# mpasha3/trips-py

Hardware: AMD Instinct MI355X
Metric: krylov_iters_per_sec (higher is better)
Workload: dtype f32; 1 GPU; blur4096_cgls; image=4096x4096 fp32, psf=Gaussian 9x9 sigma=(3,3), reflect, solver=CGLS (trips.solvers.CGLS semantics, tol=0), noise=1% Gaussian, parallelism=single

## Files before the change

trips_py_amd/csrc/blur2d.hip:

```cpp
#include "trk_internal.h"
#include <hip/hip_ext.h>

#include <cmath>
#include <cstdlib>
#include <type_traits>
#include <vector>

using namespace trk;

namespace {

constexpr int NT = 256;
constexpr int TW = 128;
constexpr int TH = 32;

typedef float f4 __attribute__((ext_vector_type(4)));

__host__ __device__ constexpr int rup4(int v) { return (v + 3) & ~3; }

__device__ __forceinline__ int reflect(int i, int n) {
  if ((unsigned)i < (unsigned)n) return i;
  const int p = 2 * n;
  i %= p;
  if (i < 0) i += p;
  return (i >= n) ? (p - 1 - i) : i;
}

enum Bc : int { BC_REFLECT = 0, BC_CONSTANT = 1, BC_NEAREST = 2, BC_MIRROR = 3, BC_WRAP = 4 };

template <int BC>
__device__ __forceinline__ int bmap(int i, int n) {
  if constexpr (BC == BC_REFLECT) {
    return reflect(i, n);
  } else {
    if ((unsigned)i < (unsigned)n) return i;
    if constexpr (BC == BC_CONSTANT) {
      return -1;
    } else if constexpr (BC == BC_NEAREST) {
      return i < 0 ? 0 : n - 1;
    } else if constexpr (BC == BC_WRAP) {
      i %= n;
      return i < 0 ? i + n : i;
    } else {
      if (n == 1) return 0;
      const int p = 2 * n - 2;
      i %= p;
      if (i < 0) i += p;
      return (i >= n) ? (p - i) : i;
    }
  }
}

template <int BC>
__device__ __forceinline__ float bload(const float* row, int j, int n) {
  const int g = bmap<BC>(j, n);
  if constexpr (BC == BC_CONSTANT)
    if (g < 0) return 0.f;
  return row[g];
}

template <class F>
int bc_dispatch(int bc, F&& f) {
  switch (bc) {
    case BC_CONSTANT: return f(std::integral_constant<int, BC_CONSTANT>{});
    case BC_NEAREST: return f(std::integral_constant<int, BC_NEAREST>{});
    case BC_MIRROR: return f(std::integral_constant<int, BC_MIRROR>{});
    case BC_WRAP: return f(std::integral_constant<int, BC_WRAP>{});
    default: return f(std::integral_constant<int, BC_REFLECT>{});
  }
}

struct BlurImpl {
  int nx, ny, kh, kw;
  int bc;
  bool separable;
  bool tiled;
  float* w_dev[2];
  float* sep_dev[2];
};

template <int KH, int KW, bool SEP, bool SUMSQ, int BC = BC_REFLECT>
__global__ __launch_bounds__(NT, (SEP && KH <= 9) ? 4 : 2) void k_blur_strip(const float* __restrict__ x, int64_t ldx, float* __restrict__ y,
                                                   int64_t ldy, int nx, int ny, const float* __restrict__ wts,
                                                   double* __restrict__ partials, int strips_x, int rows_per_band) {
  constexpr int T = KH - 1 - KH / 2;
  constexpr int L = KW - 1 - KW / 2;
  constexpr int R = KW / 2;
  constexpr int LP = rup4(L), RP = rup4(R);
  constexpr int SW = TW + LP + RP;
  constexpr int RING = TH + KH - 1;
  constexpr int OFF = LP - L;
  constexpr int NV = (OFF + KW + 3 + 3) / 4;
  constexpr int SW4 = SW / 4;
  constexpr int NPF = (TH * SW4 + NT - 1) / NT;

  __shared__ f4 S4[RING * SW4];
  float* const S = reinterpret_cast<float*>(S4);
  __shared__ double red[NT / 64];

  const int sj = blockIdx.x % strips_x, band = blockIdx.x / strips_x;
  const int j0 = sj * TW;
  const int i_begin = band * rows_per_band;
  const int i_end = (i_begin + rows_per_band < nx) ? i_begin + rows_per_band : nx;
  x += (int64_t)blockIdx.y * ldx;
  y += (int64_t)blockIdx.y * ldy;

  const bool fast = ((ny & 3) == 0) && ((reinterpret_cast<uintptr_t>(x) & 15u) == 0);

  auto load_group = [&](int rel, int c4) -> f4 {
    const int gi = bmap<BC>(i_begin - T + rel, nx);
    if constexpr (BC == BC_CONSTANT)
      if (gi < 0) return (f4){0.f, 0.f, 0.f, 0.f};
    const int gc = j0 - LP + 4 * c4;
    const float* row = x + (int64_t)gi * ny;
    if (fast && gc >= 0 && gc + 3 < ny) return *reinterpret_cast<const f4*>(row + gc);
    return (f4){bload<BC>(row, gc, ny), bload<BC>(row, gc + 1, ny), bload<BC>(row, gc + 2, ny), bload<BC>(row, gc + 3, ny)};
  };

  auto load_direct = [&](int rel0, int count) {
    for (int idx = threadIdx.x; idx < count * SW4; idx += NT) {
      const int r = idx / SW4, c4 = idx - r * SW4;
      S4[((rel0 + r) % RING) * SW4 + c4] = load_group(rel0 + r, c4);
    }
  };

  float wr[SEP ? KW : 1], wc[SEP ? KH : 1];
  if (SEP) {
#pragma unroll
    for (int b = 0; b < KW; ++b) wr[b] = wts[b];
#pragma unroll
    for (int a = 0; a < KH; ++a) wc[a] = wts[KW + a];
  }

  const int tx = threadIdx.x & 31, ty = threadIdx.x >> 5;
  const int gj = j0 + 4 * tx;
  const bool vec_ok = ((ny & 3) == 0) && ((reinterpret_cast<uintptr_t>(y) & 15u) == 0) && (j0 + TW <= ny);
  double ss = 0.0;

  load_direct(0, RING);
  int rb = 0;
  for (int i0 = i_begin; i0 < i_end; i0 += TH) {
    const int rel_base = i0 - i_begin;
    const bool has_next = (i0 + TH < i_end);
    __syncthreads();

    f4 pf[NPF];
#pragma unroll
    for (int q = 0; q < NPF; ++q) pf[q] = (f4){0.f, 0.f, 0.f, 0.f};
    if (has_next) {
#pragma unroll
      for (int q = 0; q < NPF; ++q) {
        const int idx = threadIdx.x + q * NT;
        if (idx < TH * SW4) {
          const int r = idx / SW4, c4 = idx - r * SW4;
          pf[q] = load_group(rel_base + RING + r, c4);
        }
      }
    }

    float acc[4][4];
#pragma unroll
    for (int rr = 0; rr < 4; ++rr)
#pragma unroll
      for (int c = 0; c < 4; ++c) acc[rr][c] = 0.f;
#pragma unroll
    for (int a = 0; a < KH + 3; ++a) {
      int slot = rb + 4 * ty + a;
      if (slot >= RING) slot -= RING;
      float v[NV * 4];
#pragma unroll
      for (int q = 0; q < NV; ++q) {
        const f4 t = S4[slot * SW4 + tx + q];
        v[4 * q] = t[0];
        v[4 * q + 1] = t[1];
        v[4 * q + 2] = t[2];
        v[4 * q + 3] = t[3];
      }
      if (SEP) {
        float h[4] = {0.f, 0.f, 0.f, 0.f};
#pragma unroll
        for (int b = 0; b < KW; ++b)
#pragma unroll
          for (int c = 0; c < 4; ++c) h[c] = fmaf(wr[b], v[OFF + c + b], h[c]);
#pragma unroll
        for (int rr = 0; rr < 4; ++rr) {
          if (a - rr >= 0 && a - rr < KH) {
            const float w = wc[a - rr];
#pragma unroll
            for (int c = 0; c < 4; ++c) acc[rr][c] = fmaf(w, h[c], acc[rr][c]);
          }
        }
      } else {
#pragma unroll
        for (int rr = 0; rr < 4; ++rr) {
          if (a - rr >= 0 && a - rr < KH) {
#pragma unroll
            for (int b = 0; b < KW; ++b) {
              const float w = wts[(a - rr) * KW + b];
#pragma unroll
              for (int c = 0; c < 4; ++c) acc[rr][c] = fmaf(w, v[OFF + c + b], acc[rr][c]);
            }
          }
        }
      }
    }

    if (vec_ok) {
#pragma unroll
      for (int rr = 0; rr < 4; ++rr) {
        const int gi = i0 + 4 * ty + rr;
        if (gi < i_end) {
          *reinterpret_cast<f4*>(y + (int64_t)gi * ny + gj) = (f4){acc[rr][0], acc[rr][1], acc[rr][2], acc[rr][3]};
          if (SUMSQ)
            ss += (double)acc[rr][0] * acc[rr][0] + (double)acc[rr][1] * acc[rr][1] +
                  (double)acc[rr][2] * acc[rr][2] + (double)acc[rr][3] * acc[rr][3];
        }
      }
    } else {
#pragma unroll
      for (int rr = 0; rr < 4; ++rr) {
        const int gi = i0 + 4 * ty + rr;
        if (gi < i_end) {
#pragma unroll
          for (int c = 0; c < 4; ++c)
            if (gj + c < ny) {
              y[(int64_t)gi * ny + gj + c] = acc[rr][c];
              if (SUMSQ) ss += (double)acc[rr][c] * acc[rr][c];
            }
        }
      }
    }

    if (has_next) {
      __syncthreads();
#pragma unroll
      for (int q = 0; q < NPF; ++q) {
        const int idx = threadIdx.x + q * NT;
        if (idx < TH * SW4) {
          const int r = idx / SW4, c4 = idx - r * SW4;
          S4[((rel_base + RING + r) % RING) * SW4 + c4] = pf[q];
        }
      }
      rb += TH;
      if (rb >= RING) rb -= RING;
    }
  }
  if (SUMSQ) {
    ss = block_sum<NT>(ss, red);
    if (threadIdx.x == 0) partials[(size_t)blockIdx.y * gridDim.x + blockIdx.x] = ss;
  }
}

typedef unsigned int u4 __attribute__((ext_vector_type(4)));
typedef float f2 __attribute__((ext_vector_type(2)));

__host__ __device__ constexpr int gcd_c(int a, int b) { return b == 0 ? a : gcd_c(b, a % b); }
__host__ __device__ constexpr int lcm_c(int a, int b) { return a / gcd_c(a, b) * b; }
__host__ __device__ constexpr int pmod(int a, int m) { return ((a % m) + m) % m; }

constexpr int SPAN = 256;

struct SlideFuse {
  const float* x2;
  float* comb;
  double sign;
  ScalarSrc num, den;
};

struct SlideEpi {
  const float* z;
  Coef a, b;
};

enum Rc : int { RC_NONE = 0, RC_NORM = 1, RC_RATIO = 2 };
struct SlideRatio {
  const float* z;
  float* out;
  ScalarSrc num, den;
  float sign;
  int on_z, pub_den;
  double* pub;
};

template <int KH, int KW, int D, bool SUMSQ, bool FUSE, bool EPI = false, int BC = BC_REFLECT, int RC = RC_NONE>
__global__ __launch_bounds__(64) void k_blur_slide(const float* __restrict__ x, int64_t ldx, float* __restrict__ y,
                                                   int64_t ldy, int nx, int ny, const float* __restrict__ wts,
                                                   double* __restrict__ partials, int spans_x, int nbands,
                                                   int rows_per_band, SlideFuse fz, int nt_store, SlideEpi ep = SlideEpi{},
                                                   SlideRatio rq = SlideRatio{}) {
  static_assert(RC == RC_NONE || !FUSE, "the recompute forms take one operand");
  static_assert(RC != RC_NORM || (SUMSQ && !EPI), "RC_NORM: the sum of squares alone");
  static_assert(RC != RC_RATIO || (EPI && !SUMSQ), "RC_RATIO: an epilogue form without a sum");
  constexpr int T = KH - 1 - KH / 2;
  constexpr int Lh = KW - 1 - KW / 2;
  constexpr int OFFC = 4 - Lh;
  constexpr int U = lcm_c(KH, D);
  static_assert(Lh <= 4 && KW / 2 <= 4, "sliding kernel handles halos of at most one 4-column group");

  int band, span;
  {
    const int id = blockIdx.x, total = nbands * spans_x;
    const int xcd = id & 7, local = id >> 3;
    const int t = xcd * (total >> 3) + min(xcd, total & 7) + local;
    band = t / spans_x;
    span = t - band * spans_x;
  }
  x += (int64_t)blockIdx.y * ldx;
  y += (int64_t)blockIdx.y * ldy;
  const int i_begin = band * rows_per_band;
  const int i_end = (i_begin + rows_per_band < nx) ? i_begin + rows_per_band : nx;
  const int lane = threadIdx.x;
  const int c0 = span * SPAN + 4 * lane;
  const bool active = c0 < ny;
  const int cc = active ? c0 : ny - 4;
  const int cl = (BC == BC_WRAP && c0 == 0) ? ny - 4 : (cc >= 4) ? cc - 4 : 0;
  const int cr = (BC == BC_WRAP && c0 + 4 == ny) ? 0 : (cc + 8 <= ny) ? cc + 4 : ny - 4;
  const bool ledge = (c0 == 0), redge = (c0 + 4 == ny);
  const bool edge_span = (span == 0) || ((span + 1) * SPAN >= ny);

  const unsigned img_bytes = (unsigned)nx * (unsigned)ny * 4u;
  const auto rin = __builtin_amdgcn_make_buffer_rsrc((void*)x, 0, img_bytes, 0x00020000);
  const auto rout = __builtin_amdgcn_make_buffer_rsrc((void*)(RC == RC_RATIO ? rq.out : y), 0, img_bytes, 0x00020000);
  const auto rin2 = __builtin_amdgcn_make_buffer_rsrc((void*)(FUSE ? fz.x2 : x), 0, img_bytes, 0x00020000);
  const auto rcomb = __builtin_amdgcn_make_buffer_rsrc((void*)(FUSE ? fz.comb : y), 0, img_bytes, 0x00020000);
  float cb = 0.f;
  if (FUSE) cb = (fz.sign == 0.0) ? 0.f : (float)(fz.sign * scalar_from_wave(fz.num, threadIdx.x) / scalar_from_wave(fz.den, threadIdx.x));
  const int vl = cl * 4, vr = cr * 4;
  const int vc = cc * 4;
  const int vst = c0 * 4;

  const bool up = (band & 1) != 0;
  float wr[KW], wc[KH];
#pragma unroll
  for (int b = 0; b < KW; ++b) wr[b] = wts[b];
#pragma unroll
  for (int a = 0; a < KH; ++a) wc[a] = up ? wts[KW + KH - 1 - a] : wts[KW + a];

  const int band_rows = i_end - i_begin;
  const int total = ((band_rows + KH - 1 + U - 1) / U) * U;
  const int rowbytes = ny * 4;
  const int dir = up ? -1 : 1;
  const int first = up ? (i_end - 1 + KH / 2) : (i_begin - T);
  const int last = first + dir * (total - 1);
  const bool interior = (first >= 0) && (first < nx) && (last >= 0) && (last < nx);
  const int ofirst = up ? (i_end - 1) : i_begin;

  f4 pL[D], pC[D], pR[D];
  f4 qL[FUSE ? D : 1], qC[FUSE ? D : 1], qR[FUSE ? D : 1];
  auto issue = [&](int t, int slot) {
    int gi = first + dir * t;
    if (!interior) gi = bmap<BC>(gi, nx);
    if constexpr (BC == BC_CONSTANT) {
      if (gi < 0) {
        const f4 z = (f4){0.f, 0.f, 0.f, 0.f};
        pL[slot] = pC[slot] = pR[slot] = z;
        if (FUSE) qL[slot] = qC[slot] = qR[slot] = z;
        return;
      }
    }
    const int so = gi * rowbytes;
    pL[slot] = __builtin_bit_cast(f4, __builtin_amdgcn_raw_buffer_load_b128(rin, vl, so, 0));
    pC[slot] = __builtin_bit_cast(f4, __builtin_amdgcn_raw_buffer_load_b128(rin, vc, so, 0));
    pR[slot] = __builtin_bit_cast(f4, __builtin_amdgcn_raw_buffer_load_b128(rin, vr, so, 0));
    if (FUSE) {
      qL[slot] = __builtin_bit_cast(f4, __builtin_amdgcn_raw_buffer_load_b128(rin2, vl, so, 0));
      qC[slot] = __builtin_bit_cast(f4, __builtin_amdgcn_raw_buffer_load_b128(rin2, vc, so, 0));
      qR[slot] = __builtin_bit_cast(f4, __builtin_amdgcn_raw_buffer_load_b128(rin2, vr, so, 0));
    }
  };
#pragma unroll
  for (int d = 0; d < D; ++d) issue(d, d);
  float ea = 1.f, eb = 0.f;
  f4 zq[EPI ? D : 1];
  const auto rz = __builtin_amdgcn_make_buffer_rsrc((void*)(RC == RC_RATIO ? rq.z : (EPI && ep.z) ? ep.z : x), 0, img_bytes, 0x00020000);
  const bool has_z = RC == RC_RATIO || (EPI && ep.z != nullptr);
  auto issue_z = [&](int o, int slot) {
    const int oc = o < band_rows - 1 ? o : band_rows - 1;
    zq[slot] = __builtin_bit_cast(f4, __builtin_amdgcn_raw_buffer_load_b128(rz, vc, (ofirst + dir * oc) * rowbytes, 0));
  };
  if constexpr (RC == RC_RATIO) {
#pragma unroll
    for (int d = 0; d < D; ++d) issue_z(d, d);
    const double qn = scalar_from_wave(rq.num, lane), qd = scalar_from_wave(rq.den, lane);
    const float c = rq.sign * (float)(qn / qd);
    ea = rq.on_z ? 1.f : c;
    eb = rq.on_z ? c : 1.f;
    if (blockIdx.x == 0 && blockIdx.y == 0 && lane == 0 && rq.pub) *rq.pub = rq.pub_den ? qd : qn;
  } else if (EPI) {
    ea = (float)coef_eval(ep.a);
    eb = has_z ? (float)coef_eval(ep.b) : 0.f;
    if (has_z) {
#pragma unroll
      for (int d = 0; d < D; ++d) issue_z(d, d);
    }
  }

  f2 acc[KH][2];
  double ss = 0.0;
  float qacc = 0.f;

  auto block = [&](int t0, auto guard_tag) {
    constexpr bool GUARD = decltype(guard_tag)::value;
#pragma unroll
    for (int u = 0; u < U; ++u) {
      const int t = t0 + u;
      const int slot = u % D;
      f4 Lv = pL[slot], Cv = pC[slot], Rv = pR[slot];
      if (FUSE) {
        Lv = Lv + cb * qL[slot];
        Cv = Cv + cb * qC[slot];
        Rv = Rv + cb * qR[slot];
        const int graw = first + dir * t;
        if (graw >= i_begin && graw < i_end && active)
          __builtin_amdgcn_raw_buffer_store_b128(__builtin_bit_cast(u4, Cv), rcomb, vst + graw * rowbytes, 0, 0);
      }
      if (!GUARD || t + D < total) issue(t + D, slot);
      if constexpr (BC == BC_REFLECT) {
        if (edge_span) {
          const f4 rev = (f4){Cv[3], Cv[2], Cv[1], Cv[0]};
          if (ledge) Lv = rev;
          if (redge) Rv = rev;
        }
      } else if constexpr (BC != BC_WRAP) {
        if (edge_span) {
          f4 le, re;
          if constexpr (BC == BC_CONSTANT) {
            le = re = (f4){0.f, 0.f, 0.f, 0.f};
          } else if constexpr (BC == BC_NEAREST) {
            le = (f4){Cv[0], Cv[0], Cv[0], Cv[0]};
            re = (f4){Cv[3], Cv[3], Cv[3], Cv[3]};
          } else {
            le = (f4){Rv[0], Cv[3], Cv[2], Cv[1]};
            re = (f4){Cv[2], Cv[1], Cv[0], Lv[3]};
          }
          if (ledge) Lv = le;
          if (redge) Rv = re;
        }
      }
      const float v[12] = {Lv[0], Lv[1], Lv[2], Lv[3], Cv[0], Cv[1], Cv[2], Cv[3], Rv[0], Rv[1], Rv[2], Rv[3]};
      float h0 = 0.f, h1 = 0.f, h2 = 0.f, h3 = 0.f;
#pragma unroll
      for (int b = 0; b < KW; ++b) {
        h0 = fmaf(wr[b], v[OFFC + b], h0);
        h1 = fmaf(wr[b], v[OFFC + b + 1], h1);
        h2 = fmaf(wr[b], v[OFFC + b + 2], h2);
        h3 = fmaf(wr[b], v[OFFC + b + 3], h3);
      }
      const f2 hlo = {h0, h1}, hhi = {h2, h3};
#pragma unroll
      for (int a = 0; a < KH; ++a) {
        const int k = pmod(u - a, KH);
        if (a == 0) {
          acc[k][0] = wc[0] * hlo;
          acc[k][1] = wc[0] * hhi;
        } else {
          acc[k][0] = wc[a] * hlo + acc[k][0];
          acc[k][1] = wc[a] * hhi + acc[k][1];
        }
      }
      const int o = t - (KH - 1);
      if (!GUARD || (o >= 0 && o < band_rows)) {
        const int kd = pmod(u - (KH - 1), KH);
        f4 out = (f4){acc[kd][0][0], acc[kd][0][1], acc[kd][1][0], acc[kd][1][1]};
        if (EPI) {
          const int zs = pmod(u - (KH - 1), D);
          if constexpr (RC == RC_RATIO) {
            const f4 zv = zq[zs];
            if (rq.on_z) {
#pragma unroll
              for (int e = 0; e < 4; ++e) out[e] = fmaf(eb, zv[e], out[e]);
            } else {
#pragma unroll
              for (int e = 0; e < 4; ++e) out[e] = fmaf(ea, out[e], zv[e]);
            }
            issue_z(o + D, zs);
          } else if (has_z) {
            const f4 zv = zq[zs];
#pragma unroll
            for (int e = 0; e < 4; ++e) out[e] = fmaf(ea, out[e], eb * zv[e]);
            issue_z(o + D, zs);
          } else {
#pragma unroll
            for (int e = 0; e < 4; ++e) out[e] = ea * out[e];
          }
        }
        if (active) {
          if constexpr (RC != RC_NORM) {
            if (nt_store & 1)
              __builtin_amdgcn_raw_buffer_store_b128(__builtin_bit_cast(u4, out), rout, vst + (ofirst + dir * o) * rowbytes, 0, 2);
            else
              __builtin_amdgcn_raw_buffer_store_b128(__builtin_bit_cast(u4, out), rout, vst + (ofirst + dir * o) * rowbytes, 0, 0);
          }
          if (SUMSQ) qacc = fmaf(out[0], out[0], fmaf(out[1], out[1], fmaf(out[2], out[2], fmaf(out[3], out[3], qacc))));
        }
      }
      if (SUMSQ && (u & 3) == 3) {
        ss += (double)qacc;
        qacc = 0.f;
      }
    }
  };
  block(0, std::true_type{});
  int t0 = U;
  for (; t0 + U < total; t0 += U) block(t0, std::false_type{});
  if (t0 < total) block(t0, std::true_type{});
  if (SUMSQ) ss += (double)qacc;
  if (SUMSQ) {
    ss = wave_sum(ss);
    if (lane == 0) partials[(size_t)blockIdx.y * gridDim.x + blockIdx.x] = ss;
  }
}

template <bool SUMSQ, int BC = BC_REFLECT>
__global__ __launch_bounds__(NT) void k_blur_generic(const float* __restrict__ x, int64_t ldx, float* __restrict__ y,
                                                     int64_t ldy, int nx, int ny, int kh, int kw,
                                                     const float* __restrict__ w, double* __restrict__ partials) {
  __shared__ double red[NT / 64];
  const int T = kh - 1 - kh / 2, L = kw - 1 - kw / 2;
  x += (int64_t)blockIdx.y * ldx;
  y += (int64_t)blockIdx.y * ldy;
  const int64_t npix = (int64_t)nx * ny;
  double ss = 0.0;
  for (int64_t idx = (int64_t)blockIdx.x * NT + threadIdx.x; idx < npix; idx += (int64_t)gridDim.x * NT) {
    const int i = (int)(idx / ny), j = (int)(idx - (int64_t)i * ny);
    float acc = 0.f;
    for (int a = 0; a < kh; ++a) {
      const int gi = bmap<BC>(i - T + a, nx);
      if constexpr (BC == BC_CONSTANT)
        if (gi < 0) continue;
      const float* row = x + (int64_t)gi * ny;
      for (int b = 0; b < kw; ++b) acc = fmaf(w[a * kw + b], bload<BC>(row, j - L + b, ny), acc);
    }
    y[idx] = acc;
    if (SUMSQ) ss += (double)acc * acc;
  }
  if (SUMSQ) {
    ss = block_sum<NT>(ss, red);
    if (threadIdx.x == 0) partials[(size_t)blockIdx.y * gridDim.x + blockIdx.x] = ss;
  }
}

inline void strip_grid(int nx, int ny, int batch, int* strips_x, int* rows_per_band, int* nband) {
  const int sx = ceil_div(ny, TW), steps = ceil_div(nx, TH);
  int want = (4 * cu_count()) / (sx * (batch > 0 ? batch : 1));
  if (want < 1) want = 1;
  if (want > steps) want = steps;
  const int steps_per_band = ceil_div(steps, want);
  *strips_x = sx;
  *rows_per_band = steps_per_band * TH;
  *nband = ceil_div(nx, *rows_per_band);
}

template <int K, int BC>
int launch_strip(const BlurImpl* im, int tr, const float* x, int64_t ldx, float* y, int64_t ldy, int batch,
                 double* part, int strips_x, int rows_per_band, int nband, hipStream_t s) {
  dim3 grid(strips_x * nband, batch), block(NT);
  const float* w = im->separable ? im->sep_dev[tr] : im->w_dev[tr];
#define BL(SEP, SS) \
  hipLaunchKernelGGL((k_blur_strip<K, K, SEP, SS, BC>), grid, block, 0, s, x, ldx, y, ldy, im->nx, im->ny, w, part, strips_x, rows_per_band)
  if (im->separable) { if (part) BL(true, true); else BL(true, false); }
  else               { if (part) BL(false, true); else BL(false, false); }
#undef BL
  TRK_LAUNCH_CHECK();
  return TRK_OK;
}

template <int K, int D, int BC>
int launch_slide(const BlurImpl* im, int tr, const float* x, int64_t ldx, float* y, int64_t ldy, int batch,
                 double* part, int spans_x, int nbands, int rows_per_band, hipStream_t s, hipEvent_t ev0, hipEvent_t ev1,
                 const SlideFuse* fuse = nullptr, const SlideEpi* epi = nullptr) {
  dim3 grid(spans_x * nbands, batch), block(64);
  const float* w = im->sep_dev[tr];
  const int nts = stream_nontemporal((int64_t)im->nx * im->ny);
  if (fuse) {
    hipExtLaunchKernelGGL((k_blur_slide<K, K, D, true, true, false, BC>), grid, block, 0, s, ev0, ev1, 0, x, ldx, y, ldy, im->nx, im->ny, w, part, spans_x, nbands, rows_per_band, *fuse, nts, SlideEpi{}, SlideRatio{});
    TRK_LAUNCH_CHECK();
    return TRK_OK;
  }
  const SlideFuse nofuse{nullptr, nullptr, 0.0, {nullptr, 0}, {nullptr, 0}};
  if (epi) {
    if (part)
      hipExtLaunchKernelGGL((k_blur_slide<K, K, D, true, false, true, BC>), grid, block, 0, s, ev0, ev1, 0, x, ldx, y, ldy, im->nx, im->ny, w, part, spans_x, nbands, rows_per_band, nofuse, nts, *epi, SlideRatio{});
    else
      hipExtLaunchKernelGGL((k_blur_slide<K, K, D, false, false, true, BC>), grid, block, 0, s, ev0, ev1, 0, x, ldx, y, ldy, im->nx, im->ny, w, part, spans_x, nbands, rows_per_band, nofuse, nts, *epi, SlideRatio{});
    TRK_LAUNCH_CHECK();
    return TRK_OK;
  }
  if (part)
    hipExtLaunchKernelGGL((k_blur_slide<K, K, D, true, false, false, BC>), grid, block, 0, s, ev0, ev1, 0, x, ldx, y, ldy, im->nx, im->ny, w, part, spans_x, nbands, rows_per_band, nofuse, nts, SlideEpi{}, SlideRatio{});
  else
    hipExtLaunchKernelGGL((k_blur_slide<K, K, D, false, false, false, BC>), grid, block, 0, s, ev0, ev1, 0, x, ldx, y, ldy, im->nx, im->ny, w, part, spans_x, nbands, rows_per_band, nofuse, nts, SlideEpi{}, SlideRatio{});
  TRK_LAUNCH_CHECK();
  return TRK_OK;
}

inline void slide_grid(int nx, int ny, int batch, int kh, int U, int* spans_x, int* nbands, int* rows_per_band) {
  const int sx = ceil_div(ny, SPAN);
  const double slots = 4.0 * cu_count();
  const int nb = batch > 0 ? batch : 1;
  int rows = U;
  while (rows - (kh - 1) < kh + 1) rows += U;
  int rpb = rows - (kh - 1);
  double best = 1e300;
  for (;; rows += U) {
    const int r = rows - (kh - 1);
    const double x = (double)sx * ceil_div(nx, r) * nb / slots;
    const double g = x <= 1.0 ? 1.0 : 0.6 + 0.45 * x + 0.5 * (ceil(x) - 1.0);
    const bool last = x <= 1.0 || r >= nx;
    if ((x * slots <= 3840.0 || last) && rows * g < best) {
      best = rows * g;
      rpb = r;
    }
    if (last) break;
  }
  *spans_x = sx;
  *nbands = ceil_div(nx, rpb);
  *rows_per_band = rpb;
}

inline bool slide_shape_ok(const BlurImpl* im) {
  return im->separable && im->kh == im->kw && (im->kh & 1) && im->kh >= 3 && im->kh <= 9 && (im->ny & 3) == 0 &&
         im->ny >= 8 && (int64_t)im->nx * im->ny < ((int64_t)1 << 29);
}

int blur_apply_fused(trk_op* op, int tr, const float* x1, const float* x2, double sign, ScalarSrc num, ScalarSrc den,
                     float* comb, float* y, double* partials, int cap, int* n_partials, hipStream_t s) {
  auto* im = static_cast<BlurImpl*>(op->impl);
  if (!slide_shape_ok(im) || !aligned16(x1) || !aligned16(y) || (x2 && (!aligned16(x2) || !aligned16(comb))))
    return fail(TRK_EUNSUPPORTED, "blur2d fused apply: needs a separable odd PSF <= 9x9, ny %% 4 == 0, 16-byte aligned buffers");
  if (x2 && (comb == x1 || comb == x2))
    return fail(TRK_EINVAL, "blur2d fused apply: comb must not alias an input (halo rows are shared)");
  int spans_x, nbands, rpb;
  const int Usel = (im->kh == 9) ? 9 : (im->kh == 7) ? 7 : (im->kh == 5) ? 5 : 6;
  slide_grid(im->nx, im->ny, 1, im->kh, Usel, &spans_x, &nbands, &rpb);
  const int nblk = spans_x * nbands;
  if (nblk > cap) return fail(TRK_EINVAL, "blur2d fused apply: partial buffer holds %d doubles, %d needed", cap, nblk);
  *n_partials = nblk;
  const SlideFuse fz{x2, comb, sign, num, den};
  const SlideFuse* fzp = x2 ? &fz : nullptr;
  hipEvent_t ev0 = nullptr, ev1 = nullptr;
  if (trk_timer* t = op->timer)
    if ((op->timer_which == 2 || op->timer_which == tr) && t->used < t->cap) {
      ev0 = t->ev[2 * t->used];
      ev1 = t->ev[2 * t->used + 1];
      ++t->used;
    }
  return bc_dispatch(im->bc, [&](auto bc) {
    constexpr int BC = decltype(bc)::value;
    switch (im->kh) {
      case 3: return launch_slide<3, 6, BC>(im, tr, x1, 0, y, 0, 1, partials, spans_x, nbands, rpb, s, ev0, ev1, fzp);
      case 5: return launch_slide<5, 5, BC>(im, tr, x1, 0, y, 0, 1, partials, spans_x, nbands, rpb, s, ev0, ev1, fzp);
      case 7: return launch_slide<7, 7, BC>(im, tr, x1, 0, y, 0, 1, partials, spans_x, nbands, rpb, s, ev0, ev1, fzp);
      default:
        return launch_slide<9, 9, BC>(im, tr, x1, 0, y, 0, 1, partials, spans_x, nbands, rpb, s, ev0, ev1, fzp);
    }
  });
}

int blur_apply(trk_op* op, int tr, const float* x, int64_t ldx, float* y, int64_t ldy, int batch, double* sumsq,
               hipStream_t s) {
  auto* im = static_cast<BlurImpl*>(op->impl);
  double* part = nullptr;
  int nblk;
  const bool slide_ok = slide_shape_ok(im) && aligned16(x) && aligned16(y) &&
                        (batch == 1 || ((ldx & 3) == 0 && (ldy & 3) == 0));
  if (slide_ok) {
    int spans_x, nbands, rpb;
    const int Usel = (im->kh == 9) ? 9 : (im->kh == 7) ? 7 : (im->kh == 5) ? 5 : 6;
    slide_grid(im->nx, im->ny, batch, im->kh, Usel, &spans_x, &nbands, &rpb);
    nblk = spans_x * nbands;
    if (sumsq)
      if (int rc = scratch_doubles(s, (size_t)nblk * batch, &part)) return rc;
    hipEvent_t ev0 = nullptr, ev1 = nullptr;
    if (trk_timer* t = op->timer)
      if ((op->timer_which == 2 || op->timer_which == tr) && t->used < t->cap) {
        ev0 = t->ev[2 * t->used];
        ev1 = t->ev[2 * t->used + 1];
        ++t->used;
      }
    const int rc = bc_dispatch(im->bc, [&](auto bc) {
      constexpr int BC = decltype(bc)::value;
      switch (im->kh) {
        case 3: return launch_slide<3, 6, BC>(im, tr, x, ldx, y, ldy, batch, part, spans_x, nbands, rpb, s, ev0, ev1);
        case 5: return launch_slide<5, 5, BC>(im, tr, x, ldx, y, ldy, batch, part, spans_x, nbands, rpb, s, ev0, ev1);
        case 7: return launch_slide<7, 7, BC>(im, tr, x, ldx, y, ldy, batch, part, spans_x, nbands, rpb, s, ev0, ev1);
        default: return launch_slide<9, 9, BC>(im, tr, x, ldx, y, ldy, batch, part, spans_x, nbands, rpb, s, ev0, ev1);
      }
    });
    if (rc) return rc;
    if (sumsq) return finalize_sums(part, nblk * batch, 1, 1, sumsq, s);
    return TRK_OK;
  }
  if (im->tiled) {
    int strips_x, rows_per_band, nband;
    strip_grid(im->nx, im->ny, batch, &strips_x, &rows_per_band, &nband);
    nblk = strips_x * nband;
    if (sumsq)
      if (int rc = scratch_doubles(s, (size_t)nblk * batch, &part)) return rc;
    TimerScope tm(op->timer, op->timer_which, tr, s);
    const int rc = bc_dispatch(im->bc, [&](auto bc) {
      constexpr int BC = decltype(bc)::value;
      switch (im->kh) {
        case 3: return launch_strip<3, BC>(im, tr, x, ldx, y, ldy, batch, part, strips_x, rows_per_band, nband, s);
        case 5: return launch_strip<5, BC>(im, tr, x, ldx, y, ldy, batch, part, strips_x, rows_per_band, nband, s);
        case 7: return launch_strip<7, BC>(im, tr, x, ldx, y, ldy, batch, part, strips_x, rows_per_band, nband, s);
        case 9: return launch_strip<9, BC>(im, tr, x, ldx, y, ldy, batch, part, strips_x, rows_per_band, nband, s);
        case 11: return launch_strip<11, BC>(im, tr, x, ldx, y, ldy, batch, part, strips_x, rows_per_band, nband, s);
        case 13: return launch_strip<13, BC>(im, tr, x, ldx, y, ldy, batch, part, strips_x, rows_per_band, nband, s);
        case 15: return launch_strip<15, BC>(im, tr, x, ldx, y, ldy, batch, part, strips_x, rows_per_band, nband, s);
        default: return fail(TRK_EUNSUPPORTED, "blur2d: no strip kernel for %dx%d", im->kh, im->kw);
      }
    });
    tm.stop();
    if (rc) return rc;
  } else {
    const int64_t npix = (int64_t)im->nx * im->ny;
    int64_t want = (npix + NT - 1) / NT;
    if (want > 4096) want = 4096;
    nblk = (int)(want < 1 ? 1 : want);
    if (sumsq)
      if (int rc = scratch_doubles(s, (size_t)nblk * batch, &part)) return rc;
    dim3 grid(nblk, batch);
    TimerScope tm(op->timer, op->timer_which, tr, s);
    bc_dispatch(im->bc, [&](auto bc) {
      constexpr int BC = decltype(bc)::value;
      if (part)
        hipLaunchKernelGGL((k_blur_generic<true, BC>), grid, dim3(NT), 0, s, x, ldx, y, ldy, im->nx, im->ny, im->kh, im->kw, im->w_dev[tr], part);
      else
        hipLaunchKernelGGL((k_blur_generic<false, BC>), grid, dim3(NT), 0, s, x, ldx, y, ldy, im->nx, im->ny, im->kh, im->kw, im->w_dev[tr], part);
      return 0;
    });
    tm.stop();
    TRK_LAUNCH_CHECK();
  }
  if (sumsq) return finalize_sums(part, nblk * batch, 1, 1, sumsq, s);
  return TRK_OK;
}

int blur_apply_axpby_plain(trk_op* op, int tr, const float* x, Coef a, Coef b, const float* z, float* out, double* sumsq,
                           hipStream_t s) {
  auto* im = static_cast<BlurImpl*>(op->impl);
  if (!slide_shape_ok(im) || !aligned16(x) || !aligned16(out) || (z && !aligned16(z))) return TRK_EUNSUPPORTED;
  int spans_x, nbands, rpb;
  const int Usel = (im->kh == 9) ? 9 : (im->kh == 7) ? 7 : (im->kh == 5) ? 5 : 6;
  slide_grid(im->nx, im->ny, 1, im->kh, Usel, &spans_x, &nbands, &rpb);
  const int nblk = spans_x * nbands;
  double* part = nullptr;
  if (sumsq)
    if (int rc = scratch_doubles(s, (size_t)nblk, &part)) return rc;
  hipEvent_t ev0 = nullptr, ev1 = nullptr;
  if (trk_timer* t = op->timer)
    if ((op->timer_which == 2 || op->timer_which == tr) && t->used < t->cap) {
      ev0 = t->ev[2 * t->used];
      ev1 = t->ev[2 * t->used + 1];
      ++t->used;
    }
  const SlideEpi ep{z, a, b};
  const int rc = bc_dispatch(im->bc, [&](auto bc) {
    constexpr int BC = decltype(bc)::value;
    switch (im->kh) {
      case 3: return launch_slide<3, 6, BC>(im, tr, x, 0, out, 0, 1, part, spans_x, nbands, rpb, s, ev0, ev1, nullptr, &ep);
      case 5: return launch_slide<5, 5, BC>(im, tr, x, 0, out, 0, 1, part, spans_x, nbands, rpb, s, ev0, ev1, nullptr, &ep);
      case 7: return launch_slide<7, 7, BC>(im, tr, x, 0, out, 0, 1, part, spans_x, nbands, rpb, s, ev0, ev1, nullptr, &ep);
      default: return launch_slide<9, 9, BC>(im, tr, x, 0, out, 0, 1, part, spans_x, nbands, rpb, s, ev0, ev1, nullptr, &ep);
    }
  });
  if (rc) return rc;
  if (sumsq) return finalize_sums(part, nblk, 1, 1, sumsq, s);
  return TRK_OK;
}

template <int K, int D, int BC>
int launch_slide_rc(const BlurImpl* im, int tr, const float* x, double* part, const SlideRatio* rq, int spans_x, int nbands,
                    int rows_per_band, hipStream_t s, hipEvent_t ev0, hipEvent_t ev1) {
  dim3 grid(spans_x * nbands, 1), block(64);
  const float* w = im->sep_dev[tr];
  const SlideFuse nofuse{nullptr, nullptr, 0.0, {nullptr, 0}, {nullptr, 0}};
  if (rq)
    hipExtLaunchKernelGGL((k_blur_slide<K, K, D, false, false, true, BC, RC_RATIO>), grid, block, 0, s, ev0, ev1, 0, x, 0, rq->out, 0, im->nx, im->ny, w, part, spans_x, nbands, rows_per_band, nofuse, 0, SlideEpi{}, *rq);
  else
    hipExtLaunchKernelGGL((k_blur_slide<K, K, D, true, false, false, BC, RC_NORM>), grid, block, 0, s, ev0, ev1, 0, x, 0, (float*)nullptr, 0, im->nx, im->ny, w, part, spans_x, nbands, rows_per_band, nofuse, 0, SlideEpi{}, SlideRatio{});
  TRK_LAUNCH_CHECK();
  return TRK_OK;
}

int blur_apply_rc(trk_op* op, int tr, const float* x, double* partials, int cap, int* n_partials, const SlideRatio* rq, hipStream_t s) {
  auto* im = static_cast<BlurImpl*>(op->impl);
  if (!slide_shape_ok(im) || !aligned16(x) || (rq && (!aligned16(rq->z) || !aligned16(rq->out))))
    return fail(TRK_EUNSUPPORTED, "blur2d recompute forms: need a separable odd PSF <= 9x9, ny %% 4 == 0, 16-byte aligned buffers");
  if (rq && (rq->out == x || rq->z == x))
    return fail(TRK_EINVAL, "blur2d ratio apply: out / z must not alias x (halo rows are shared)");
  int spans_x, nbands, rpb;
  const int Usel = (im->kh == 9) ? 9 : (im->kh == 7) ? 7 : (im->kh == 5) ? 5 : 6;
  slide_grid(im->nx, im->ny, 1, im->kh, Usel, &spans_x, &nbands, &rpb);
  if (!rq) {
    const int nblk = spans_x * nbands;
    if (nblk > cap) return fail(TRK_EINVAL, "blur2d norm-only apply: partial buffer holds %d doubles, %d needed", cap, nblk);
    *n_partials = nblk;
  }
  hipEvent_t ev0 = nullptr, ev1 = nullptr;
  if (trk_timer* t = op->timer)
    if (rq && (op->timer_which == 2 || op->timer_which == tr) && t->used < t->cap) {
      ev0 = t->ev[2 * t->used];
      ev1 = t->ev[2 * t->used + 1];
      ++t->used;
    }
  return bc_dispatch(im->bc, [&](auto bc) {
    constexpr int BC = decltype(bc)::value;
    switch (im->kh) {
      case 3: return launch_slide_rc<3, 6, BC>(im, tr, x, partials, rq, spans_x, nbands, rpb, s, ev0, ev1);
      case 5: return launch_slide_rc<5, 5, BC>(im, tr, x, partials, rq, spans_x, nbands, rpb, s, ev0, ev1);
      case 7: return launch_slide_rc<7, 7, BC>(im, tr, x, partials, rq, spans_x, nbands, rpb, s, ev0, ev1);
      default: return launch_slide_rc<9, 9, BC>(im, tr, x, partials, rq, spans_x, nbands, rpb, s, ev0, ev1);
    }
  });
}

int blur_apply_norm(trk_op* op, int tr, const float* x, double* partials, int cap, int* n_partials, hipStream_t s) {
  return blur_apply_rc(op, tr, x, partials, cap, n_partials, nullptr, s);
}

int blur_apply_ratio(trk_op* op, int tr, const float* x, const RatioCoef& c, const float* z, float* out, hipStream_t s) {
  const SlideRatio rq{z, out, c.num, c.den, (float)c.sign, c.on_z, c.pub_den, c.pub};
  return blur_apply_rc(op, tr, x, nullptr, 0, nullptr, &rq, s);
}

void blur_destroy(trk_op* op) {
  auto* im = static_cast<BlurImpl*>(op->impl);
  for (int t = 0; t < 2; ++t) {
    if (im->w_dev[t]) (void)hipFree(im->w_dev[t]);
    if (im->sep_dev[t]) (void)hipFree(im->sep_dev[t]);
  }
  delete im;
}

}

namespace trk {
bool blur_separable_params(trk_op* op, int* nx, int* ny, int* kh, int* kw, const float** sep_fwd, const float** sep_adj,
                           int* boundary) {
  if (!op || op->kind != 1) return false;
  auto* im = static_cast<BlurImpl*>(op->impl);
  if (!im->separable || !im->sep_dev[0] || !im->sep_dev[1]) return false;
  if (boundary) *boundary = im->bc;
  *nx = im->nx;
  *ny = im->ny;
  *kh = im->kh;
  *kw = im->kw;
  *sep_fwd = im->sep_dev[0];
  *sep_adj = im->sep_dev[1];
  return true;
}
}

extern "C" int trk_blur2d_create(const double* psf, int kh, int kw, int nx, int ny, trk_op** out) {
  return trk_blur2d_create_bc(psf, kh, kw, nx, ny, TRK_BOUNDARY_REFLECT, out);
}

extern "C" int trk_blur2d_create_bc(const double* psf, int kh, int kw, int nx, int ny, int boundary, trk_op** out) {
  TRK_REQUIRE(psf && out, "trk_blur2d_create: NULL argument");
  TRK_REQUIRE(kh >= 1 && kw >= 1 && nx >= 1 && ny >= 1, "trk_blur2d_create: sizes must be >= 1");
  TRK_REQUIRE((int64_t)kh * kw <= (1 << 24), "trk_blur2d_create: PSF too large");
  TRK_REQUIRE(boundary >= TRK_BOUNDARY_REFLECT && boundary <= TRK_BOUNDARY_WRAP, "trk_blur2d_create_bc: unknown boundary mode %d", boundary);
  static_assert(TRK_BOUNDARY_REFLECT == BC_REFLECT && TRK_BOUNDARY_CONSTANT == BC_CONSTANT && TRK_BOUNDARY_NEAREST == BC_NEAREST &&
                    TRK_BOUNDARY_MIRROR == BC_MIRROR && TRK_BOUNDARY_WRAP == BC_WRAP,
                "blur2d boundary modes follow trk.h");
  auto* im = new BlurImpl{nx, ny, kh, kw, boundary, false, false, {nullptr, nullptr}, {nullptr, nullptr}};

  std::vector<float> wf((size_t)kh * kw), wt((size_t)kh * kw);
  for (int a = 0; a < kh; ++a)
    for (int b = 0; b < kw; ++b) {
      wf[(size_t)a * kw + b] = (float)psf[(size_t)(kh - 1 - a) * kw + (kw - 1 - b)];
      wt[(size_t)a * kw + b] = (float)psf[(size_t)a * kw + b];
    }

  int pa = 0, pb = 0;
  double pmax = 0.0;
  for (int a = 0; a < kh; ++a)
    for (int b = 0; b < kw; ++b)
      if (std::fabs(psf[(size_t)a * kw + b]) > pmax) {
        pmax = std::fabs(psf[(size_t)a * kw + b]);
        pa = a;
        pb = b;
      }
  std::vector<double> col(kh), row(kw);
  bool sep = pmax > 0.0;
  if (sep) {
    const double piv = psf[(size_t)pa * kw + pb];
    for (int a = 0; a < kh; ++a) col[a] = psf[(size_t)a * kw + pb];
    for (int b = 0; b < kw; ++b) row[b] = psf[(size_t)pa * kw + b] / piv;
    for (int a = 0; a < kh && sep; ++a)
      for (int b = 0; b < kw; ++b)
        if (std::fabs(psf[(size_t)a * kw + b] - col[a] * row[b]) > 1e-12 * pmax) {
          sep = false;
          break;
        }
  }
  im->separable = sep;
  im->tiled = (kh == kw) && (kh & 1) && kh >= 3 && kh <= 15;

  auto upload = [](const std::vector<float>& h, float** d) -> int {
    TRK_HIP(hipMalloc(d, h.size() * sizeof(float)));
    TRK_HIP(hipMemcpy(*d, h.data(), h.size() * sizeof(float), hipMemcpyHostToDevice));
    return TRK_OK;
  };
  int rc = upload(wf, &im->w_dev[0]);
  if (!rc) rc = upload(wt, &im->w_dev[1]);
  if (!rc && sep) {
    std::vector<float> sf(kw + kh), st(kw + kh);
    for (int b = 0; b < kw; ++b) {
      sf[b] = (float)row[kw - 1 - b];
      st[b] = (float)row[b];
    }
    for (int a = 0; a < kh; ++a) {
      sf[kw + a] = (float)col[kh - 1 - a];
      st[kw + a] = (float)col[a];
    }
    rc = upload(sf, &im->sep_dev[0]);
    if (!rc) rc = upload(st, &im->sep_dev[1]);
  }
  if (rc) {
    trk_op tmp{1, 0, 0, im, nullptr, nullptr, nullptr, 0};
    blur_destroy(&tmp);
    return rc;
  }
  const int64_t n = (int64_t)nx * ny;
  auto* op = new trk_op{1, n, n, im, blur_apply, blur_destroy, nullptr, 0};
  if (slide_shape_ok(im)) op->apply_fused = blur_apply_fused;
  if (slide_shape_ok(im)) op->apply_axpby_plain = blur_apply_axpby_plain;
  if (slide_shape_ok(im)) {
    op->apply_norm = blur_apply_norm;
    op->apply_ratio = blur_apply_ratio;
  }
  *out = op;
  return TRK_OK;
}
```

Measured before the change: 8516 iters/s.

## Add lean norm-only 9x9 slide kernel with packed FMAs and border specialization

Adds an RC_NORM_LEAN variant of the sliding blur kernel for the norm-only pass with a 9x9 PSF. It precomputes the next-row load offsets for each unrolled block and issues the loads after the horizontal pass behind a sched_barrier. The horizontal filter uses packed f2 FMAs, built from v_pk_mov op_sel shuffles, instead of scalar FMAs. Interior spans run a specialization that skips the boundary-fixup and active checks. The variant is chosen only when the grid is at most four blocks per CU. It aims to cut VALU and address work and improve latency hiding in the norm-only recompute pass, at the cost of code size and inline asm.

```diff
diff --git a/trips_py_amd/csrc/blur2d.hip b/trips_py_amd/csrc/blur2d.hip
--- a/trips_py_amd/csrc/blur2d.hip
+++ b/trips_py_amd/csrc/blur2d.hip
@@ -272,7 +272,7 @@
   Coef a, b;
 };
 
-enum Rc : int { RC_NONE = 0, RC_NORM = 1, RC_RATIO = 2 };
+enum Rc : int { RC_NONE = 0, RC_NORM = 1, RC_RATIO = 2, RC_NORM_LEAN = 3 };
 struct SlideRatio {
   const float* z;
   float* out;
@@ -282,6 +282,12 @@
   double* pub;
 };
 
+__device__ __forceinline__ f2 pair_hi_lo(f2 a, f2 b) {
+  f2 d;
+  asm("v_pk_mov_b32 %0, %1, %2 op_sel:[1,0]" : "=v"(d) : "v"(a), "v"(b));
+  return d;
+}
+
 template <int KH, int KW, int D, bool SUMSQ, bool FUSE, bool EPI = false, int BC = BC_REFLECT, int RC = RC_NONE>
 __global__ __launch_bounds__(64) void k_blur_slide(const float* __restrict__ x, int64_t ldx, float* __restrict__ y,
                                                    int64_t ldy, int nx, int ny, const float* __restrict__ wts,
@@ -289,11 +295,14 @@
                                                    int rows_per_band, SlideFuse fz, int nt_store, SlideEpi ep = SlideEpi{},
                                                    SlideRatio rq = SlideRatio{}) {
   static_assert(RC == RC_NONE || !FUSE, "the recompute forms take one operand");
-  static_assert(RC != RC_NORM || (SUMSQ && !EPI), "RC_NORM: the sum of squares alone");
+  constexpr bool NORM = RC == RC_NORM || RC == RC_NORM_LEAN;
+  static_assert(!NORM || (SUMSQ && !EPI), "RC_NORM: the sum of squares alone");
+  static_assert(RC != RC_NORM_LEAN || (KH == 9 && BC != BC_CONSTANT), "the lean norm-only form: 9x9, not constant mode");
   static_assert(RC != RC_RATIO || (EPI && !SUMSQ), "RC_RATIO: an epilogue form without a sum");
   constexpr int T = KH - 1 - KH / 2;
   constexpr int Lh = KW - 1 - KW / 2;
   constexpr int OFFC = 4 - Lh;
+  constexpr bool LEAN = RC == RC_NORM_LEAN;
   constexpr int U = lcm_c(KH, D);
   static_assert(Lh <= 4 && KW / 2 <= 4, "sliding kernel handles halos of at most one 4-column group");
 
@@ -368,6 +377,16 @@
       qR[slot] = __builtin_bit_cast(f4, __builtin_amdgcn_raw_buffer_load_b128(rin2, vr, so, 0));
     }
   };
+  auto row_offset = [&](int t) {
+    int gi = first + dir * t;
+    if (!interior) gi = bmap<BC>(gi, nx);
+    return gi * rowbytes;
+  };
+  auto issue_at = [&](int so, int slot) {
+    pL[slot] = __builtin_bit_cast(f4, __builtin_amdgcn_raw_buffer_load_b128(rin, vl, so, 0));
+    pC[slot] = __builtin_bit_cast(f4, __builtin_amdgcn_raw_buffer_load_b128(rin, vc, so, 0));
+    pR[slot] = __builtin_bit_cast(f4, __builtin_amdgcn_raw_buffer_load_b128(rin, vr, so, 0));
+  };
 #pragma unroll
   for (int d = 0; d < D; ++d) issue(d, d);
   float ea = 1.f, eb = 0.f;
@@ -399,8 +418,14 @@
   double ss = 0.0;
   float qacc = 0.f;
 
-  auto block = [&](int t0, auto guard_tag) {
+  auto block = [&](int t0, auto guard_tag, auto border_tag) __attribute__((always_inline)) {
     constexpr bool GUARD = decltype(guard_tag)::value;
+    constexpr bool BORDER = decltype(border_tag)::value;
+    int so_next[LEAN ? U : 1];
+    if constexpr (LEAN) {
+#pragma unroll
+      for (int u = 0; u < U; ++u) so_next[u] = (!GUARD || t0 + u + D < total) ? row_offset(t0 + u + D) : 0;
+    }
 #pragma unroll
     for (int u = 0; u < U; ++u) {
       const int t = t0 + u;
@@ -414,8 +439,10 @@
         if (graw >= i_begin && graw < i_end && active)
           __builtin_amdgcn_raw_buffer_store_b128(__builtin_bit_cast(u4, Cv), rcomb, vst + graw * rowbytes, 0, 0);
       }
-      if (!GUARD || t + D < total) issue(t + D, slot);
-      if constexpr (BC == BC_REFLECT) {
+      if constexpr (!LEAN)
+        if (!GUARD || t + D < total) issue(t + D, slot);
+      if constexpr (!BORDER) {
+      } else if constexpr (BC == BC_REFLECT) {
         if (edge_span) {
           const f4 rev = (f4){Cv[3], Cv[2], Cv[1], Cv[0]};
           if (ledge) Lv = rev;
@@ -437,16 +464,40 @@
           if (redge) Rv = re;
         }
       }
-      const float v[12] = {Lv[0], Lv[1], Lv[2], Lv[3], Cv[0], Cv[1], Cv[2], Cv[3], Rv[0], Rv[1], Rv[2], Rv[3]};
-      float h0 = 0.f, h1 = 0.f, h2 = 0.f, h3 = 0.f;
-#pragma unroll
-      for (int b = 0; b < KW; ++b) {
-        h0 = fmaf(wr[b], v[OFFC + b], h0);
-        h1 = fmaf(wr[b], v[OFFC + b + 1], h1);
-        h2 = fmaf(wr[b], v[OFFC + b + 2], h2);
-        h3 = fmaf(wr[b], v[OFFC + b + 3], h3);
-      }
-      const f2 hlo = {h0, h1}, hhi = {h2, h3};
+      f2 hlo, hhi;
+      if constexpr (LEAN) {
+        const f2 ev[6] = {__builtin_shufflevector(Lv, Lv, 0, 1), __builtin_shufflevector(Lv, Lv, 2, 3),
+                          __builtin_shufflevector(Cv, Cv, 0, 1), __builtin_shufflevector(Cv, Cv, 2, 3),
+                          __builtin_shufflevector(Rv, Rv, 0, 1), __builtin_shufflevector(Rv, Rv, 2, 3)};
+        f2 od[5];
+#pragma unroll
+        for (int q = 0; q < 5; ++q)
+          if (2 * q + 1 >= OFFC && 2 * q + 1 <= OFFC + KW + 1) od[q] = pair_hi_lo(ev[q], ev[q + 1]);
+        hlo = hhi = (f2){0.f, 0.f};
+#pragma unroll
+        for (int b = 0; b < KW; ++b) {
+          const int j = OFFC + b;
+          const f2 w = {wr[b], wr[b]};
+          hlo = __builtin_elementwise_fma(w, (j & 1) ? od[j >> 1] : ev[j >> 1], hlo);
+          hhi = __builtin_elementwise_fma(w, (j & 1) ? od[(j + 2) >> 1] : ev[(j + 2) >> 1], hhi);
+        }
+      } else {
+        const float v[12] = {Lv[0], Lv[1], Lv[2], Lv[3], Cv[0], Cv[1], Cv[2], Cv[3], Rv[0], Rv[1], Rv[2], Rv[3]};
+        float h0 = 0.f, h1 = 0.f, h2 = 0.f, h3 = 0.f;
+#pragma unroll
+        for (int b = 0; b < KW; ++b) {
+          h0 = fmaf(wr[b], v[OFFC + b], h0);
+          h1 = fmaf(wr[b], v[OFFC + b + 1], h1);
+          h2 = fmaf(wr[b], v[OFFC + b + 2], h2);
+          h3 = fmaf(wr[b], v[OFFC + b + 3], h3);
+        }
+        hlo = (f2){h0, h1};
+        hhi = (f2){h2, h3};
+      }
+      if constexpr (LEAN) {
+        __builtin_amdgcn_sched_barrier(0);
+        if (!GUARD || t + D < total) issue_at(so_next[u], slot);
+      }
 #pragma unroll
       for (int a = 0; a < KH; ++a) {
         const int k = pmod(u - a, KH);
@@ -484,8 +535,8 @@
             for (int e = 0; e < 4; ++e) out[e] = ea * out[e];
           }
         }
-        if (active) {
-          if constexpr (RC != RC_NORM) {
+        if (!BORDER || active) {
+          if constexpr (!NORM) {
             if (nt_store & 1)
               __builtin_amdgcn_raw_buffer_store_b128(__builtin_bit_cast(u4, out), rout, vst + (ofirst + dir * o) * rowbytes, 0, 2);
             else
@@ -500,10 +551,18 @@
       }
     }
   };
-  block(0, std::true_type{});
-  int t0 = U;
-  for (; t0 + U < total; t0 += U) block(t0, std::false_type{});
-  if (t0 < total) block(t0, std::true_type{});
+  auto march = [&](auto border_tag) __attribute__((always_inline)) {
+    block(0, std::true_type{}, border_tag);
+    int t0 = U;
+    for (; t0 + U < total; t0 += U) block(t0, std::false_type{}, border_tag);
+    if (t0 < total) block(t0, std::true_type{}, border_tag);
+  };
+  if constexpr (LEAN && BC != BC_WRAP) {
+    if (edge_span) march(std::true_type{});
+    else march(std::false_type{});
+  } else {
+    march(std::true_type{});
+  }
   if (SUMSQ) ss += (double)qacc;
   if (SUMSQ) {
     ss = wave_sum(ss);
@@ -778,8 +837,16 @@
   const SlideFuse nofuse{nullptr, nullptr, 0.0, {nullptr, 0}, {nullptr, 0}};
   if (rq)
     hipExtLaunchKernelGGL((k_blur_slide<K, K, D, false, false, true, BC, RC_RATIO>), grid, block, 0, s, ev0, ev1, 0, x, 0, rq->out, 0, im->nx, im->ny, w, part, spans_x, nbands, rows_per_band, nofuse, 0, SlideEpi{}, *rq);
-  else
-    hipExtLaunchKernelGGL((k_blur_slide<K, K, D, true, false, false, BC, RC_NORM>), grid, block, 0, s, ev0, ev1, 0, x, 0, (float*)nullptr, 0, im->nx, im->ny, w, part, spans_x, nbands, rows_per_band, nofuse, 0, SlideEpi{}, SlideRatio{});
+  else {
+    bool lean = false;
+    if constexpr (K == 9 && BC != BC_CONSTANT) lean = spans_x * nbands <= 4 * cu_count();
+    if constexpr (K == 9 && BC != BC_CONSTANT) {
+      if (lean)
+        hipExtLaunchKernelGGL((k_blur_slide<K, K, D, true, false, false, BC, RC_NORM_LEAN>), grid, block, 0, s, ev0, ev1, 0, x, 0, (float*)nullptr, 0, im->nx, im->ny, w, part, spans_x, nbands, rows_per_band, nofuse, 0, SlideEpi{}, SlideRatio{});
+    }
+    if (!lean)
+      hipExtLaunchKernelGGL((k_blur_slide<K, K, D, true, false, false, BC, RC_NORM>), grid, block, 0, s, ev0, ev1, 0, x, 0, (float*)nullptr, 0, im->nx, im->ny, w, part, spans_x, nbands, rows_per_band, nofuse, 0, SlideEpi{}, SlideRatio{});
+  }
   TRK_LAUNCH_CHECK();
   return TRK_OK;
 }
```

Result: faster. 8711 iters/s, median of 6 (+2.3%).
